# kubeflow/Code-Intelligence

Measured on AMD Instinct MI355X. Metric: LM tokens/sec (whole node), higher is better.
Workload: dtype bf16; 1 GPU; model=AWD-LSTM 4x2400 emb800 vocab60000, global_batch=512, seq_len=512, parallelism=dp1, device=MI355X

## Files before the change

code_intelligence_amd/ops/crossentropy.py:

```python
from __future__ import annotations

import os

import torch
from torch import Tensor

from . import extension as ext

__all__ = ["tied_decoder_ce", "TiedDecoderCE"]

_EMPTY = {}


def _empty_f32(device) -> Tensor:
    key = str(device)
    if key not in _EMPTY:
        _EMPTY[key] = torch.empty(0, dtype=torch.float32, device=device)
    return _EMPTY[key]


def _fp8r_enabled() -> bool:
    return os.environ.get("CI_CE_FP8R", "1") == "1"


_STORE = 448.0

_ce_side = None


def _ce_side_stream():
    global _ce_side
    if _ce_side is None:
        _ce_side = torch.cuda.Stream()
    return _ce_side


def _ce_overlap_enabled() -> bool:
    return os.environ.get("CI_CE_2STREAM", "0") == "1"


class _FusedCEFp8Function(torch.autograd.Function):

    @staticmethod
    def forward(ctx, h: Tensor, weight: Tensor, bias: Tensor, targets: Tensor):
        lib = ext.require()
        f8 = torch.float8_e4m3fn
        N, H = h.shape
        V = weight.shape[0]
        C = int(os.environ.get("CI_CE_CHUNK", _FusedCEFunction.CHUNK))
        dev = h.device
        lse = torch.empty(N, dtype=torch.float32, device=dev)
        tgt_logit = torch.empty(N, dtype=torch.float32, device=dev)
        b32 = bias.to(torch.float32) if bias is not None else _empty_f32(dev)
        tgt64 = targets.to(torch.int64)
        sa = (h.detach().abs().amax().float() / 448.0).clamp_min(1e-12)
        sw = (weight.detach().abs().amax().float() / 448.0).clamp_min(1e-12)
        h8 = torch.empty(h.shape, dtype=f8, device=dev)
        lib.quantize_e4m3(h.detach().contiguous(), h8, sa)
        w8 = torch.empty(weight.shape, dtype=f8, device=dev)
        lib.quantize_e4m3(weight.detach().contiguous(), w8, sw)
        w8_t = w8.t()
        w_t = weight.t()
        logits_full = None
        if os.environ.get("CI_CE_SAVE_LOGITS", "1") != "0":
            try:
                logits_full = torch.empty(N, V, dtype=h.dtype, device=dev)
            except torch.cuda.OutOfMemoryError:
                pass
        scratch = None if logits_full is not None else \
            torch.empty(min(C, N), V, dtype=h.dtype, device=dev)
        for s in range(0, N, C):
            e = min(N, s + C)
            logits = logits_full[s:e] if logits_full is not None \
                else scratch[: e - s]
            if (e - s) % 16 == 0 and H % 16 == 0 and V % 16 == 0:
                torch._scaled_mm(h8[s:e], w8_t, scale_a=sa, scale_b=sw,
                                 out_dtype=h.dtype, out=logits)
            else:
                torch.mm(h[s:e], w_t, out=logits)
            lib.ce_rowstats(logits, tgt64[s:e], b32, lse[s:e],
                            tgt_logit[s:e])
        wrows = weight.detach()[tgt64]
        tgt_logit = (h.detach() * wrows).sum(dim=1, dtype=torch.float32)
        if bias is not None:
            tgt_logit = tgt_logit + b32[tgt64]
        loss = (lse - tgt_logit).mean()
        ctx.save_for_backward(h, weight, b32, tgt64, lse, w8, sw)
        ctx.logits_full = logits_full
        ctx.has_bias = bias is not None
        ctx.bias_dtype = bias.dtype if bias is not None else None
        return loss

    @staticmethod
    def backward(ctx, dloss: Tensor):
        lib = ext.require()
        f8 = torch.float8_e4m3fn
        h, weight, b32, targets, lse, w8, sw = ctx.saved_tensors
        logits_full = ctx.logits_full
        ctx.logits_full = None
        has_bias = ctx.has_bias
        N, H = h.shape
        V = weight.shape[0]
        C = _FusedCEFunction.CHUNK
        dev = h.device
        dh = torch.empty_like(h)
        scale = (dloss / N).to(torch.float32).reshape(1)
        sc_over_store = (scale.reshape(()) / _STORE)
        scratch8 = torch.empty(min(C, N), V, dtype=f8, device=dev)
        Haug = H + 16 if has_bias else H
        h_aug = h
        if has_bias:
            h_aug = torch.zeros(N, Haug, dtype=h.dtype, device=dev)
            h_aug[:, :H] = h
            h_aug[:, H] = 1
        dw_aug = torch.zeros(V, Haug, dtype=torch.float32, device=dev)
        recompute = None if logits_full is not None else \
            torch.empty(min(C, N), V, dtype=h.dtype, device=dev)
        w8_cm = w8.t().contiguous().t()
        w_t = weight.t()
        bias_arg = b32 if has_bias else _empty_f32(dev)
        overlap = _ce_overlap_enabled() and logits_full is not None
        side = _ce_side_stream() if overlap else None
        main = torch.cuda.current_stream() if overlap else None
        for s in range(0, N, C):
            e = min(N, s + C)
            c = e - s
            if logits_full is not None:
                dlog = logits_full[s:e]
            else:
                dlog = recompute[:c]
                torch.mm(h[s:e], w_t, out=dlog)
            lib.ce_dlogits_dual(dlog, targets[s:e], bias_arg, lse[s:e],
                                scale, scratch8, _STORE)
            if c % 16 == 0 and H % 16 == 0 and V % 16 == 0:
                torch._scaled_mm(scratch8[:c], w8_cm, scale_a=sc_over_store,
                                 scale_b=sw, out_dtype=h.dtype, out=dh[s:e])
            else:
                torch.mm(dlog, weight, out=dh[s:e])
            if overlap:
                side.wait_stream(main)
                with torch.cuda.stream(side):
                    dw_aug += torch.mm(dlog.t(), h_aug[s:e])
            else:
                dw_aug += torch.mm(dlog.t(), h_aug[s:e])
        if overlap:
            main.wait_stream(side)
        dw = dw_aug[:, :H]
        db = dw_aug[:, H] if has_bias else None
        return (dh, dw.to(weight.dtype),
                db.to(ctx.bias_dtype) if has_bias else None, None)


class _FusedCEFunction(torch.autograd.Function):
    CHUNK = int(os.environ.get("CI_CE_CHUNK", "65536"))

    @staticmethod
    def forward(ctx, h: Tensor, weight: Tensor, bias: Tensor, targets: Tensor):
        lib = ext.require()
        N, H = h.shape
        V = weight.shape[0]
        C = int(os.environ.get("CI_CE_CHUNK", _FusedCEFunction.CHUNK))
        lse = torch.empty(N, dtype=torch.float32, device=h.device)
        tgt_logit = torch.empty(N, dtype=torch.float32, device=h.device)
        b32 = bias.to(torch.float32) if bias is not None else _empty_f32(h.device)
        tgt64 = targets.to(torch.int64)
        save_logits = os.environ.get("CI_CE_SAVE_LOGITS", "1") != "0"
        logits_full = None
        if save_logits:
            try:
                logits_full = torch.empty(N, V, dtype=h.dtype, device=h.device)
            except torch.cuda.OutOfMemoryError:
                logits_full = None
        scratch = None if logits_full is not None else \
            torch.empty(min(C, N), V, dtype=h.dtype, device=h.device)
        w_t = weight.t()
        for s in range(0, N, C):
            e = min(N, s + C)
            logits = logits_full[s:e] if logits_full is not None \
                else scratch[: e - s]
            torch.mm(h[s:e], w_t, out=logits)
            lib.ce_rowstats(logits, tgt64[s:e], b32, lse[s:e], tgt_logit[s:e])
        loss = (lse - tgt_logit).mean()
        ctx.save_for_backward(h, weight, b32, tgt64, lse)
        ctx.logits_full = logits_full
        ctx.has_bias = bias is not None
        ctx.bias_dtype = bias.dtype if bias is not None else None
        return loss

    @staticmethod
    def backward(ctx, dloss: Tensor):
        lib = ext.require()
        h, weight, b32, targets, lse = ctx.saved_tensors
        logits_full = ctx.logits_full
        ctx.logits_full = None
        has_bias = ctx.has_bias
        N, H = h.shape
        V = weight.shape[0]
        C = _FusedCEFunction.CHUNK
        dh = torch.empty_like(h)
        scale = (dloss / N).to(torch.float32).reshape(1)
        scratch = None if logits_full is not None else \
            torch.empty(min(C, N), V, dtype=h.dtype, device=h.device)
        w_t = weight.t()
        bias_arg = b32 if has_bias else _empty_f32(h.device)
        Haug = H + 16 if has_bias else H
        h_aug = h
        if has_bias:
            h_aug = torch.zeros(N, Haug, dtype=h.dtype, device=h.device)
            h_aug[:, :H] = h
            h_aug[:, H] = 1
        dw_aug = torch.zeros(V, Haug, dtype=torch.float32, device=h.device)
        for s in range(0, N, C):
            e = min(N, s + C)
            if logits_full is not None:
                dlog = logits_full[s:e]
            else:
                dlog = scratch[: e - s]
                torch.mm(h[s:e], w_t, out=dlog)
            lib.ce_dlogits(dlog, targets[s:e], bias_arg, lse[s:e], scale)
            torch.mm(dlog, weight, out=dh[s:e])
            dw_aug += torch.mm(dlog.t(), h_aug[s:e])
        dw = dw_aug[:, :H]
        db = dw_aug[:, H] if has_bias else None
        return (dh, dw.to(weight.dtype),
                db.to(ctx.bias_dtype) if has_bias else None, None)


@torch.no_grad()
def tied_decoder_accuracy(h: Tensor, weight: Tensor, bias: Tensor | None,
                          targets: Tensor, chunk: int = 16384) -> Tensor:
    h2 = h.reshape(-1, h.shape[-1])
    t2 = targets.reshape(-1)
    w_t = weight.t()
    correct = torch.zeros((), dtype=torch.long, device=h.device)
    for s in range(0, h2.shape[0], chunk):
        e = min(h2.shape[0], s + chunk)
        logits = torch.mm(h2[s:e], w_t)
        if bias is not None:
            logits += bias
        correct += (logits.argmax(dim=1) == t2[s:e]).sum()
    return correct.float() / max(1, h2.shape[0])


def tied_decoder_ce(h: Tensor, weight: Tensor, bias: Tensor | None,
                    targets: Tensor) -> Tensor:
    if h.is_cuda:
        if _fp8r_enabled() and h.dtype == torch.bfloat16 \
                and torch.is_grad_enabled() and h.requires_grad:
            return _FusedCEFp8Function.apply(h, weight, bias, targets)
        return _FusedCEFunction.apply(h, weight, bias, targets)
    logits = torch.nn.functional.linear(h.float(), weight.float(),
                                        bias.float() if bias is not None else None)
    return torch.nn.functional.cross_entropy(logits, targets)


class TiedDecoderCE(torch.nn.Module):

    def __init__(self, decoder: torch.nn.Linear):
        super().__init__()
        self.decoder = decoder

    def forward(self, h: Tensor, targets: Tensor) -> Tensor:
        return tied_decoder_ce(h.reshape(-1, h.shape[-1]), self.decoder.weight,
                               self.decoder.bias, targets.reshape(-1))
```

code_intelligence_amd/ops/csrc/bindings.cpp:

```cpp
#include <torch/extension.h>
#include <string>
#include <vector>

namespace ci {
void lstm_seq_forward_lib(at::Tensor xp, at::Tensor bias, at::Tensor h0,
                          at::Tensor c0, at::Tensor w_hh, at::Tensor hs,
                          at::Tensor cs, at::Tensor gates);
void lstm_seq_forward_fused(at::Tensor xp, at::Tensor bias, at::Tensor h0,
                            at::Tensor c0, at::Tensor w_hh, at::Tensor hs,
                            at::Tensor cs, at::Tensor gates);
void lstm_seq_forward_lib_fp8(at::Tensor xp, at::Tensor bias, at::Tensor h0,
                              at::Tensor c0, at::Tensor w8, at::Tensor wscale,
                              at::Tensor hs, at::Tensor cs, at::Tensor gates);
void quantize_e4m3(at::Tensor src, at::Tensor dst, at::Tensor scale);
void lstm_seq_forward_gemv(at::Tensor xp, at::Tensor bias, at::Tensor h0,
                           at::Tensor c0, at::Tensor w_hh, at::Tensor hs,
                           at::Tensor cs, at::Tensor gates);
long lstm_seq_forward_gemv_persistent(at::Tensor xp, at::Tensor bias,
                                      at::Tensor h0, at::Tensor c0,
                                      at::Tensor w_hh, at::Tensor hs,
                                      at::Tensor cs, at::Tensor gates,
                                      at::Tensor ws);
void lstm_seq_forward_gemv_fp8(at::Tensor xp, at::Tensor bias, at::Tensor h0,
                               at::Tensor c0, at::Tensor w8, at::Tensor wscale,
                               at::Tensor hs, at::Tensor cs, at::Tensor gates);
void lstm_seq_backward(at::Tensor dhs, at::Tensor dhT, at::Tensor dcT,
                       at::Tensor gates, at::Tensor hs, at::Tensor cs,
                       at::Tensor c0, at::Tensor w_hh, at::Tensor dgates,
                       at::Tensor dh0, at::Tensor dc0);
at::Tensor concat_pool(at::Tensor hidden, at::Tensor lengths);
std::vector<at::Tensor> qrnn_fo_pool_fwd(at::Tensor gates, at::Tensor c0);
std::vector<at::Tensor> qrnn_fo_pool_bwd(at::Tensor gates, at::Tensor c,
                                         at::Tensor c0, at::Tensor dh,
                                         at::Tensor dcT);
void ce_rowstats(at::Tensor logits, at::Tensor targets, at::Tensor bias,
                 at::Tensor lse, at::Tensor tgt);
void ce_dlogits(at::Tensor logits, at::Tensor targets, at::Tensor bias,
                at::Tensor lse, at::Tensor scale);
void ce_dlogits_dual(at::Tensor logits, at::Tensor targets, at::Tensor bias,
                     at::Tensor lse, at::Tensor scale, at::Tensor scratch8,
                     double store_scale);
at::Tensor artar_forward(at::Tensor out, at::Tensor r);
std::vector<at::Tensor> artar_backward(at::Tensor out, at::Tensor r,
                                       at::Tensor dloss, double ca, double cb);
void fused_adamw(std::vector<at::Tensor> params, std::vector<at::Tensor> grads,
                 std::vector<at::Tensor> masters, std::vector<at::Tensor> eas_,
                 std::vector<at::Tensor> eass, double lr, double b1, double b2,
                 double eps, double wd, double bc1, double bc2);
at::Tensor emb_gather(at::Tensor weight, at::Tensor ids, at::Tensor rowmask);
std::vector<std::string> tokenize_core(const std::string& text);
std::vector<std::vector<std::string>> tokenize_core_batch(
    const std::vector<std::string>& texts);
at::Tensor emb_scatter(at::Tensor gout, at::Tensor ids, at::Tensor rowmask,
                       long V, long pad_idx);
at::Tensor dropconnect_apply(at::Tensor w, long seed, double p);
void dropconnect_grad_(at::Tensor g, long seed, double p);
}

PYBIND11_MODULE(TORCH_EXTENSION_NAME, m) {
  m.def("lstm_seq_forward_lib", &ci::lstm_seq_forward_lib,
        "LSTM sequence forward (hipBLASLt GEMM + pointwise cell kernel)");
  m.def("lstm_seq_forward_fused", &ci::lstm_seq_forward_fused,
        "LSTM sequence forward (fused MFMA cell kernel)");
  m.def("lstm_seq_forward_lib_fp8", &ci::lstm_seq_forward_lib_fp8,
        "LSTM sequence forward (fp8 recurrent scaled_mm + pointwise cell)");
  m.def("quantize_e4m3", &ci::quantize_e4m3,
        "one-pass e4m3 quantize: dst = e4m3(src/scale)");
  m.def("lstm_seq_forward_gemv", &ci::lstm_seq_forward_gemv,
        "LSTM sequence forward (fused GEMV+cell kernel, small batch)");
  m.def("lstm_seq_forward_gemv_persistent",
        &ci::lstm_seq_forward_gemv_persistent,
        "whole-sequence persistent GEMV+cell kernel (grid barrier)");
  m.def("lstm_seq_forward_gemv_fp8", &ci::lstm_seq_forward_gemv_fp8,
        "LSTM sequence forward (fp8-weight GEMV+cell kernel)");
  m.def("lstm_seq_backward", &ci::lstm_seq_backward,
        "LSTM sequence backward (pointwise + per-step GEMM)");
  m.def("concat_pool", &ci::concat_pool, "masked mean/max/last concat pool");
  m.def("qrnn_fo_pool_fwd", &ci::qrnn_fo_pool_fwd,
        "QRNN fo-pool forward scan (activates gates in place)");
  m.def("qrnn_fo_pool_bwd", &ci::qrnn_fo_pool_bwd,
        "QRNN fo-pool backward scan (pre-activation gate grads)");
  m.def("ce_rowstats", &ci::ce_rowstats, "CE row logsumexp + target logit");
  m.def("ce_dlogits", &ci::ce_dlogits, "in-place (softmax-onehot)*scale");
  m.def("ce_dlogits_dual", &ci::ce_dlogits_dual,
        "in-place bf16 dlogits + e4m3 scratch copy for the fp8 dh GEMM");
  m.def("artar_forward", &ci::artar_forward,
        "fused AR/TAR partial sums (one pass over out and r)");
  m.def("artar_backward", &ci::artar_backward,
        "fused AR/TAR gradient kernel (dout and dr in one pass)");
  m.def("fused_adamw", &ci::fused_adamw, "fused AdamW step");
  m.def("emb_gather", &ci::emb_gather, "embedding gather with row dropout");
  m.def("tokenize_core", &ci::tokenize_core, "native ASCII tokenizer core");
  m.def("tokenize_core_batch", &ci::tokenize_core_batch,
        "native ASCII tokenizer core (batch, GIL released)");
  m.def("emb_scatter", &ci::emb_scatter, "embedding grad scatter-add");
  m.def("dropconnect_apply", &ci::dropconnect_apply,
        "seeded DropConnect mask-scale (no mask tensor)");
  m.def("dropconnect_grad_", &ci::dropconnect_grad_,
        "in-place seeded DropConnect grad mask");
}
```

code_intelligence_amd/ops/csrc/ce.hip:

```cpp
#include "common.h"

#include <hip/hip_fp8.h>

namespace ci {

typedef float f32x4 __attribute__((ext_vector_type(4)));

template <typename T, int VEC>
static __device__ __forceinline__ void load_vec(const T* p, float* out) {
  T buf[VEC];
  *reinterpret_cast<int4*>(buf) = *reinterpret_cast<const int4*>(p);
  #pragma unroll
  for (int e = 0; e < VEC; ++e) out[e] = ld(buf + e);
}

template <int VEC>
static __device__ __forceinline__ void load_bias(const float* b, float* out) {
  #pragma unroll
  for (int e = 0; e < VEC; e += 4)
    *reinterpret_cast<f32x4*>(out + e) = *reinterpret_cast<const f32x4*>(b + e);
}

template <typename T, int THREADS, bool HAS_BIAS>
__global__ void ce_rowstats_kernel(const T* __restrict__ logits, long row_stride,
                                   const long* __restrict__ targets,
                                   const float* __restrict__ bias,
                                   float* __restrict__ lse,
                                   float* __restrict__ tgt, int V) {
  constexpr int NW = THREADS / kWave;
  constexpr int VEC = 16 / sizeof(T);
  const int row = blockIdx.x;
  const T* x = logits + (long)row * row_stride;
  __shared__ float red_m[NW];
  __shared__ float red_s[NW];
  const int Vv = V / VEC * VEC;
  float v8[VEC], b8[VEC];
  float m = -3.4e38f, sum = 0.f;
  for (int v = threadIdx.x * VEC; v < Vv; v += THREADS * VEC) {
    load_vec<T, VEC>(x + v, v8);
    if (HAS_BIAS) {
      load_bias<VEC>(bias + v, b8);
      #pragma unroll
      for (int e = 0; e < VEC; ++e) v8[e] += b8[e];
    }
    float bm = v8[0];
    #pragma unroll
    for (int e = 1; e < VEC; ++e) bm = fmaxf(bm, v8[e]);
    if (bm > m) {
      sum *= __expf(m - bm);
      m = bm;
    }
    #pragma unroll
    for (int e = 0; e < VEC; ++e) sum += __expf(v8[e] - m);
  }
  for (int v = Vv + threadIdx.x; v < V; v += THREADS) {
    const float val = ld(x + v) + (HAS_BIAS ? bias[v] : 0.f);
    if (val > m) {
      sum *= __expf(m - val);
      m = val;
    }
    sum += __expf(val - m);
  }
  #pragma unroll
  for (int off = kWave / 2; off > 0; off >>= 1) {
    const float om = __shfl_down(m, off);
    const float os = __shfl_down(sum, off);
    const float nm = fmaxf(m, om);
    sum = sum * __expf(m - nm) + os * __expf(om - nm);
    m = nm;
  }
  if ((threadIdx.x & (kWave - 1)) == 0) {
    red_m[threadIdx.x / kWave] = m;
    red_s[threadIdx.x / kWave] = sum;
  }
  __syncthreads();
  if (threadIdx.x == 0) {
    float gm = red_m[0];
    for (int w = 1; w < NW; ++w) gm = fmaxf(gm, red_m[w]);
    float gs = 0.f;
    for (int w = 0; w < NW; ++w) gs += red_s[w] * __expf(red_m[w] - gm);
    lse[row] = gm + __logf(gs);
    tgt[row] = ld(x + targets[row]) + (HAS_BIAS ? bias[targets[row]] : 0.f);
  }
}

void ce_rowstats(at::Tensor logits, at::Tensor targets, at::Tensor bias,
                 at::Tensor lse, at::Tensor tgt) {
  CI_CHECK_CUDA(logits); CI_CHECK_CONTIG(logits);
  const int N = logits.size(0), V = logits.size(1);
  constexpr int THREADS = 256;
  const bool hb = bias.numel() > 0;
  CI_DISPATCH_FB(logits.scalar_type(), "ce_rowstats", [&] {
    if (hb) {
      hipLaunchKernelGGL((ce_rowstats_kernel<scalar_t, THREADS, true>), dim3(N),
          dim3(THREADS), 0, stream(),
          reinterpret_cast<const scalar_t*>(logits.data_ptr()), (long)V,
          targets.data_ptr<long>(), bias.data_ptr<float>(),
          lse.data_ptr<float>(), tgt.data_ptr<float>(), V);
    } else {
      hipLaunchKernelGGL((ce_rowstats_kernel<scalar_t, THREADS, false>), dim3(N),
          dim3(THREADS), 0, stream(),
          reinterpret_cast<const scalar_t*>(logits.data_ptr()), (long)V,
          targets.data_ptr<long>(), nullptr,
          lse.data_ptr<float>(), tgt.data_ptr<float>(), V);
    }
  });
}

template <typename T, int THREADS, bool HAS_BIAS>
__global__ void ce_dlogits_kernel(T* __restrict__ logits, long row_stride,
                                  const long* __restrict__ targets,
                                  const float* __restrict__ bias,
                                  const float* __restrict__ lse,
                                  const float* __restrict__ scale, int V) {
  constexpr int VEC = 16 / sizeof(T);
  const int row = blockIdx.x;
  T* x = logits + (long)row * row_stride;
  const float l = lse[row];
  const float sc = scale[0];
  const int tgt = (int)targets[row];
  const int Vv = V / VEC * VEC;
  float v8[VEC], b8[VEC];
  for (int v = threadIdx.x * VEC; v < Vv; v += THREADS * VEC) {
    load_vec<T, VEC>(x + v, v8);
    if (HAS_BIAS) {
      load_bias<VEC>(bias + v, b8);
      #pragma unroll
      for (int e = 0; e < VEC; ++e) v8[e] += b8[e];
    }
    T buf[VEC];
    #pragma unroll
    for (int e = 0; e < VEC; ++e) {
      float p = __expf(v8[e] - l);
      if (v + e == tgt) p -= 1.f;
      st(buf + e, p * sc);
    }
    *reinterpret_cast<int4*>(x + v) = *reinterpret_cast<const int4*>(buf);
  }
  for (int v = Vv + threadIdx.x; v < V; v += THREADS) {
    float p = __expf(ld(x + v) + (HAS_BIAS ? bias[v] : 0.f) - l);
    if (v == tgt) p -= 1.f;
    st(x + v, p * sc);
  }
}

void ce_dlogits(at::Tensor logits, at::Tensor targets, at::Tensor bias,
                at::Tensor lse, at::Tensor scale) {
  CI_CHECK_CUDA(logits); CI_CHECK_CONTIG(logits);
  const int N = logits.size(0), V = logits.size(1);
  constexpr int THREADS = 256;
  const bool hb = bias.numel() > 0;
  CI_DISPATCH_FB(logits.scalar_type(), "ce_dlogits", [&] {
    if (hb) {
      hipLaunchKernelGGL((ce_dlogits_kernel<scalar_t, THREADS, true>),
          dim3(N), dim3(THREADS), 0, stream(),
          reinterpret_cast<scalar_t*>(logits.data_ptr()), (long)V,
          targets.data_ptr<long>(), bias.data_ptr<float>(),
          lse.data_ptr<float>(), scale.data_ptr<float>(), V);
    } else {
      hipLaunchKernelGGL((ce_dlogits_kernel<scalar_t, THREADS, false>),
          dim3(N), dim3(THREADS), 0, stream(),
          reinterpret_cast<scalar_t*>(logits.data_ptr()), (long)V,
          targets.data_ptr<long>(), nullptr,
          lse.data_ptr<float>(), scale.data_ptr<float>(), V);
    }
  });
}

template <typename T, int THREADS, bool HAS_BIAS>
__global__ void ce_dlogits_dual_kernel(T* __restrict__ logits, long row_stride,
                                       const long* __restrict__ targets,
                                       const float* __restrict__ bias,
                                       const float* __restrict__ lse,
                                       const float* __restrict__ scale,
                                       unsigned char* __restrict__ scratch8,
                                       long srs, float store_scale, int V) {
  constexpr int VEC = 16 / sizeof(T);
  const int row = blockIdx.x;
  T* x = logits + (long)row * row_stride;
  unsigned char* s8 = scratch8 + (long)row * srs;
  const float l = lse[row];
  const float sc = scale[0];
  const int tgt = (int)targets[row];
  const int Vv = V / VEC * VEC;
  float v8[VEC], b8[VEC];
  for (int v = threadIdx.x * VEC; v < Vv; v += THREADS * VEC) {
    load_vec<T, VEC>(x + v, v8);
    if (HAS_BIAS) {
      load_bias<VEC>(bias + v, b8);
      #pragma unroll
      for (int e = 0; e < VEC; ++e) v8[e] += b8[e];
    }
    T buf[VEC];
    unsigned char q8[VEC];
    #pragma unroll
    for (int e = 0; e < VEC; ++e) {
      float p = __expf(v8[e] - l);
      if (v + e == tgt) p -= 1.f;
      st(buf + e, p * sc);
      q8[e] = __hip_fp8_e4m3(p * store_scale).__x;
    }
    *reinterpret_cast<int4*>(x + v) = *reinterpret_cast<const int4*>(buf);
    if constexpr (VEC == 8) {
      *reinterpret_cast<uint2*>(s8 + v) = *reinterpret_cast<const uint2*>(q8);
    } else {
      *reinterpret_cast<unsigned int*>(s8 + v) =
          *reinterpret_cast<const unsigned int*>(q8);
    }
  }
  for (int v = Vv + threadIdx.x; v < V; v += THREADS) {
    float p = __expf(ld(x + v) + (HAS_BIAS ? bias[v] : 0.f) - l);
    if (v == tgt) p -= 1.f;
    st(x + v, p * sc);
    s8[v] = __hip_fp8_e4m3(p * store_scale).__x;
  }
}

void ce_dlogits_dual(at::Tensor logits, at::Tensor targets, at::Tensor bias,
                     at::Tensor lse, at::Tensor scale, at::Tensor scratch8,
                     double store_scale) {
  CI_CHECK_CUDA(logits); CI_CHECK_CONTIG(logits); CI_CHECK_CONTIG(scratch8);
  const int N = logits.size(0), V = logits.size(1);
  TORCH_CHECK(scratch8.size(0) >= N && scratch8.size(1) == V,
              "ce_dlogits_dual: scratch too small");
  TORCH_CHECK(scratch8.scalar_type() == at::ScalarType::Byte ||
              scratch8.scalar_type() == at::ScalarType::Float8_e4m3fn);
  constexpr int THREADS = 256;
  const bool hb = bias.numel() > 0;
  CI_DISPATCH_FB(logits.scalar_type(), "ce_dlogits_dual", [&] {
    if (hb) {
      hipLaunchKernelGGL((ce_dlogits_dual_kernel<scalar_t, THREADS, true>),
          dim3(N), dim3(THREADS), 0, stream(),
          reinterpret_cast<scalar_t*>(logits.data_ptr()), (long)V,
          targets.data_ptr<long>(), bias.data_ptr<float>(),
          lse.data_ptr<float>(), scale.data_ptr<float>(),
          reinterpret_cast<unsigned char*>(scratch8.data_ptr()),
          (long)V, (float)store_scale, V);
    } else {
      hipLaunchKernelGGL((ce_dlogits_dual_kernel<scalar_t, THREADS, false>),
          dim3(N), dim3(THREADS), 0, stream(),
          reinterpret_cast<scalar_t*>(logits.data_ptr()), (long)V,
          targets.data_ptr<long>(), nullptr,
          lse.data_ptr<float>(), scale.data_ptr<float>(),
          reinterpret_cast<unsigned char*>(scratch8.data_ptr()),
          (long)V, (float)store_scale, V);
    }
  });
}

}
```

Before: 620,200 tokens/s.

## Fuse CE row logsumexp and dlogits into one forward pass with register-cached rows

Adds a kernel that reads each logits row once into registers, computes the logsumexp, and writes the bf16 dlogits in place along with an e4m3 copy during forward. The scale is 1/N, and the dloss multiply is deferred to the weight/bias gradients. Backward then skips the dlogits kernel and uses the stored fp8 buffer directly, removing a second full read/write pass over the N×V logits. In exchange it allocates an extra N×V fp8 buffer, uses heavy register caching (32 uint4 per thread) that may cut occupancy, and assumes dloss only scales the output. The dh GEMM still applies the dloss scale, while dw now gets it from an explicit post-multiply.

Measured after the change: 627,600 tokens/s, median of 6. 1.01x the previous value.

```diff
diff --git a/code_intelligence_amd/ops/crossentropy.py b/code_intelligence_amd/ops/crossentropy.py
--- a/code_intelligence_amd/ops/crossentropy.py
+++ b/code_intelligence_amd/ops/crossentropy.py
@@ -24,6 +24,8 @@
 
 
 _STORE = 448.0
+
+_ONEPASS_MAX_V = 256 * 32 * 8
 
 _ce_side = None
 
@@ -67,6 +69,18 @@
                 logits_full = torch.empty(N, V, dtype=h.dtype, device=dev)
             except torch.cuda.OutOfMemoryError:
                 pass
+        dlog8_full = None
+        if logits_full is not None and V <= _ONEPASS_MAX_V \
+                and H % 16 == 0 and V % 16 == 0 \
+                and N % 16 == 0 and min(C, N) % 16 == 0:
+            try:
+                dlog8_full = torch.empty(N, V, dtype=f8, device=dev)
+            except torch.cuda.OutOfMemoryError:
+                pass
+        onepass = dlog8_full is not None
+        if onepass:
+            inv_n = (torch.ones((), dtype=torch.float32, device=dev)
+                     / N).reshape(1)
         scratch = None if logits_full is not None else \
             torch.empty(min(C, N), V, dtype=h.dtype, device=dev)
         for s in range(0, N, C):
@@ -78,8 +92,12 @@
                                  out_dtype=h.dtype, out=logits)
             else:
                 torch.mm(h[s:e], w_t, out=logits)
-            lib.ce_rowstats(logits, tgt64[s:e], b32, lse[s:e],
-                            tgt_logit[s:e])
+            if onepass:
+                lib.ce_onepass_dual(logits, tgt64[s:e], b32, lse[s:e],
+                                    inv_n, dlog8_full[s:e], _STORE)
+            else:
+                lib.ce_rowstats(logits, tgt64[s:e], b32, lse[s:e],
+                                tgt_logit[s:e])
         wrows = weight.detach()[tgt64]
         tgt_logit = (h.detach() * wrows).sum(dim=1, dtype=torch.float32)
         if bias is not None:
@@ -87,6 +105,8 @@
         loss = (lse - tgt_logit).mean()
         ctx.save_for_backward(h, weight, b32, tgt64, lse, w8, sw)
         ctx.logits_full = logits_full
+        ctx.dlog8_full = dlog8_full
+        ctx.chunk = C
         ctx.has_bias = bias is not None
         ctx.bias_dtype = bias.dtype if bias is not None else None
         return loss
@@ -98,15 +118,19 @@
         h, weight, b32, targets, lse, w8, sw = ctx.saved_tensors
         logits_full = ctx.logits_full
         ctx.logits_full = None
+        dlog8_full = ctx.dlog8_full
+        ctx.dlog8_full = None
+        onepass = dlog8_full is not None
         has_bias = ctx.has_bias
         N, H = h.shape
         V = weight.shape[0]
-        C = _FusedCEFunction.CHUNK
+        C = ctx.chunk if onepass else _FusedCEFunction.CHUNK
         dev = h.device
         dh = torch.empty_like(h)
         scale = (dloss / N).to(torch.float32).reshape(1)
         sc_over_store = (scale.reshape(()) / _STORE)
-        scratch8 = torch.empty(min(C, N), V, dtype=f8, device=dev)
+        scratch8 = None if onepass else \
+            torch.empty(min(C, N), V, dtype=f8, device=dev)
         Haug = H + 16 if has_bias else H
         h_aug = h
         if has_bias:
@@ -130,10 +154,14 @@
             else:
                 dlog = recompute[:c]
                 torch.mm(h[s:e], w_t, out=dlog)
-            lib.ce_dlogits_dual(dlog, targets[s:e], bias_arg, lse[s:e],
-                                scale, scratch8, _STORE)
+            if onepass:
+                dlog8 = dlog8_full[s:e]
+            else:
+                lib.ce_dlogits_dual(dlog, targets[s:e], bias_arg, lse[s:e],
+                                    scale, scratch8, _STORE)
+                dlog8 = scratch8[:c]
             if c % 16 == 0 and H % 16 == 0 and V % 16 == 0:
-                torch._scaled_mm(scratch8[:c], w8_cm, scale_a=sc_over_store,
+                torch._scaled_mm(dlog8, w8_cm, scale_a=sc_over_store,
                                  scale_b=sw, out_dtype=h.dtype, out=dh[s:e])
             else:
                 torch.mm(dlog, weight, out=dh[s:e])
@@ -147,6 +175,12 @@
             main.wait_stream(side)
         dw = dw_aug[:, :H]
         db = dw_aug[:, H] if has_bias else None
+        if onepass:
+            dl = dloss.to(torch.float32)
+            dw_out = torch.empty(V, H, dtype=weight.dtype, device=dev)
+            torch.mul(dw, dl, out=dw_out)
+            return (dh, dw_out,
+                    (db * dl).to(ctx.bias_dtype) if has_bias else None, None)
         return (dh, dw.to(weight.dtype),
                 db.to(ctx.bias_dtype) if has_bias else None, None)
 
diff --git a/code_intelligence_amd/ops/csrc/bindings.cpp b/code_intelligence_amd/ops/csrc/bindings.cpp
--- a/code_intelligence_amd/ops/csrc/bindings.cpp
+++ b/code_intelligence_amd/ops/csrc/bindings.cpp
@@ -39,6 +39,9 @@
                 at::Tensor lse, at::Tensor scale);
 void ce_dlogits_dual(at::Tensor logits, at::Tensor targets, at::Tensor bias,
                      at::Tensor lse, at::Tensor scale, at::Tensor scratch8,
+                     double store_scale);
+void ce_onepass_dual(at::Tensor logits, at::Tensor targets, at::Tensor bias,
+                     at::Tensor lse, at::Tensor scale, at::Tensor out8,
                      double store_scale);
 at::Tensor artar_forward(at::Tensor out, at::Tensor r);
 std::vector<at::Tensor> artar_backward(at::Tensor out, at::Tensor r,
@@ -84,6 +87,8 @@
   m.def("ce_dlogits", &ci::ce_dlogits, "in-place (softmax-onehot)*scale");
   m.def("ce_dlogits_dual", &ci::ce_dlogits_dual,
         "in-place bf16 dlogits + e4m3 scratch copy for the fp8 dh GEMM");
+  m.def("ce_onepass_dual", &ci::ce_onepass_dual,
+        "one read of the row: lse + in-place bf16 dlogits + e4m3 copy");
   m.def("artar_forward", &ci::artar_forward,
         "fused AR/TAR partial sums (one pass over out and r)");
   m.def("artar_backward", &ci::artar_backward,
diff --git a/code_intelligence_amd/ops/csrc/ce.hip b/code_intelligence_amd/ops/csrc/ce.hip
--- a/code_intelligence_amd/ops/csrc/ce.hip
+++ b/code_intelligence_amd/ops/csrc/ce.hip
@@ -248,4 +248,185 @@
   });
 }
 
-}
+constexpr int kOnepassMaxVec = 32;
+
+static __device__ __forceinline__ void unpack_bf16x8(const uint4& c,
+                                                     float* out) {
+  out[0] = __uint_as_float(c.x << 16); out[1] = __uint_as_float(c.x & 0xffff0000u);
+  out[2] = __uint_as_float(c.y << 16); out[3] = __uint_as_float(c.y & 0xffff0000u);
+  out[4] = __uint_as_float(c.z << 16); out[5] = __uint_as_float(c.z & 0xffff0000u);
+  out[6] = __uint_as_float(c.w << 16); out[7] = __uint_as_float(c.w & 0xffff0000u);
+}
+
+template <int THREADS, bool HAS_BIAS>
+__global__ __launch_bounds__(THREADS) void ce_onepass_dual_kernel(
+    __hip_bfloat16* __restrict__ logits, long row_stride,
+    const long* __restrict__ targets, const float* __restrict__ bias,
+    float* __restrict__ lse, const float* __restrict__ scale,
+    unsigned char* __restrict__ out8, long srs, float store_scale, int V) {
+  #pragma clang fp contract(off)
+  using T = __hip_bfloat16;
+  constexpr int NW = THREADS / kWave;
+  constexpr int VEC = 8;
+  const int row = blockIdx.x;
+  T* x = logits + (long)row * row_stride;
+  unsigned char* s8 = out8 + (long)row * srs;
+  __shared__ float red_m[NW];
+  __shared__ float red_s[NW];
+  __shared__ float lse_sh;
+  const int Vv = V / VEC * VEC;
+  uint4 cache[kOnepassMaxVec];
+  #pragma unroll
+  for (int k = 0; k < kOnepassMaxVec; ++k) {
+    const int v = (threadIdx.x + k * THREADS) * VEC;
+    cache[k] = *reinterpret_cast<const uint4*>(x + min(v, Vv - VEC));
+  }
+  #pragma unroll
+  for (int k = 0; k < kOnepassMaxVec; ++k)
+    asm volatile("" : "+v"(cache[k].x), "+v"(cache[k].y), "+v"(cache[k].z),
+                      "+v"(cache[k].w));
+  float v8[VEC], b8[VEC];
+  float m = -3.4e38f, sum = 0.f;
+  #pragma unroll
+  for (int k = 0; k < kOnepassMaxVec; ++k) {
+    const int v = (threadIdx.x + k * THREADS) * VEC;
+    if (v < Vv) {
+      unpack_bf16x8(cache[k], v8);
+      if (HAS_BIAS) {
+        load_bias<VEC>(bias + v, b8);
+        #pragma unroll
+        for (int e = 0; e < VEC; ++e) v8[e] += b8[e];
+      }
+      float bm = v8[0];
+      #pragma unroll
+      for (int e = 1; e < VEC; ++e) bm = fmaxf(bm, v8[e]);
+      if (bm > m) {
+        sum *= __expf(m - bm);
+        m = bm;
+      }
+      #pragma unroll
+      for (int e = 0; e < VEC; ++e) sum += __expf(v8[e] - m);
+    }
+  }
+  for (int v = Vv + threadIdx.x; v < V; v += THREADS) {
+    const float val = ld(x + v) + (HAS_BIAS ? bias[v] : 0.f);
+    if (val > m) {
+      sum *= __expf(m - val);
+      m = val;
+    }
+    sum += __expf(val - m);
+  }
+  #pragma unroll
+  for (int off = kWave / 2; off > 0; off >>= 1) {
+    const float om = __shfl_down(m, off);
+    const float os = __shfl_down(sum, off);
+    const float nm = fmaxf(m, om);
+    const float t = os * __expf(om - nm);
+    sum = off > 1 ? __builtin_fmaf(sum, __expf(m - nm), t)
+                  : sum * __expf(m - nm) + t;
+    m = nm;
+  }
+  if ((threadIdx.x & (kWave - 1)) == 0) {
+    red_m[threadIdx.x / kWave] = m;
+    red_s[threadIdx.x / kWave] = sum;
+  }
+  __syncthreads();
+  if (threadIdx.x == 0) {
+    float gm = red_m[0];
+    for (int w = 1; w < NW; ++w) gm = fmaxf(gm, red_m[w]);
+    float gs = 0.f;
+    for (int w = 0; w < NW; ++w) gs += red_s[w] * __expf(red_m[w] - gm);
+    const float r = gm + __logf(gs);
+    lse[row] = r;
+    lse_sh = r;
+  }
+  __syncthreads();
+  #pragma unroll
+  for (int k = 0; k < kOnepassMaxVec; ++k)
+    asm volatile("" : "+v"(cache[k].x), "+v"(cache[k].y), "+v"(cache[k].z),
+                      "+v"(cache[k].w));
+  const float* bias2 = bias;
+  asm volatile("" : "+s"(bias2));
+  const float l = lse_sh;
+  const float sc = scale[0];
+  const int tgt = (int)targets[row];
+  #pragma unroll
+  for (int k = 0; k < kOnepassMaxVec; ++k) {
+    const int v = (threadIdx.x + k * THREADS) * VEC;
+    if (v < Vv) {
+      unpack_bf16x8(cache[k], v8);
+      if (HAS_BIAS) {
+        load_bias<VEC>(bias2 + v, b8);
+        #pragma unroll
+        for (int e = 0; e < VEC; ++e) v8[e] += b8[e];
+      }
+      T buf[VEC];
+      unsigned char q8[VEC];
+      #pragma unroll
+      for (int e = 0; e < VEC; ++e) {
+        float p = __expf(v8[e] - l);
+        if (v + e == tgt) p -= 1.f;
+        st(buf + e, p * sc);
+        q8[e] = __hip_fp8_e4m3(p * store_scale).__x;
+      }
+      *reinterpret_cast<int4*>(x + v) = *reinterpret_cast<const int4*>(buf);
+      *reinterpret_cast<uint2*>(s8 + v) = *reinterpret_cast<const uint2*>(q8);
+    }
+  }
+  for (int v = Vv + threadIdx.x; v < V; v += THREADS) {
+    float p = __expf(ld(x + v) + (HAS_BIAS ? bias2[v] : 0.f) - l);
+    if (v == tgt) p -= 1.f;
+    st(x + v, p * sc);
+    s8[v] = __hip_fp8_e4m3(p * store_scale).__x;
+  }
+}
+
+void ce_onepass_dual(at::Tensor logits, at::Tensor targets, at::Tensor bias,
+                     at::Tensor lse, at::Tensor scale, at::Tensor out8,
+                     double store_scale) {
+  CI_CHECK_CUDA(logits); CI_CHECK_CONTIG(logits); CI_CHECK_CONTIG(out8);
+  CI_CHECK_CUDA(targets); CI_CHECK_CUDA(lse); CI_CHECK_CUDA(scale);
+  CI_CHECK_CUDA(out8);
+  TORCH_CHECK(logits.dim() == 2 && out8.dim() == 2);
+  TORCH_CHECK(logits.scalar_type() == at::ScalarType::BFloat16,
+              "ce_onepass_dual: bf16 logits only");
+  constexpr int THREADS = 256;
+  const int N = logits.size(0), V = logits.size(1);
+  TORCH_CHECK(V >= 8, "ce_onepass_dual: V must hold one 16-byte vector");
+  TORCH_CHECK(V / 8 <= kOnepassMaxVec * THREADS,
+              "ce_onepass_dual: V=", V, " exceeds the register-cached row (",
+              kOnepassMaxVec * THREADS * 8, ")");
+  TORCH_CHECK(out8.size(0) >= N && out8.size(1) == V,
+              "ce_onepass_dual: fp8 output too small");
+  TORCH_CHECK(out8.scalar_type() == at::ScalarType::Byte ||
+              out8.scalar_type() == at::ScalarType::Float8_e4m3fn);
+  TORCH_CHECK(targets.scalar_type() == at::ScalarType::Long &&
+              targets.numel() >= N && lse.numel() >= N &&
+              lse.scalar_type() == at::ScalarType::Float &&
+              scale.scalar_type() == at::ScalarType::Float &&
+              scale.numel() >= 1);
+  const bool hb = bias.numel() > 0;
+  TORCH_CHECK(!hb || (bias.is_cuda() && bias.numel() >= V &&
+                      bias.scalar_type() == at::ScalarType::Float));
+  if (N == 0) return;
+  using T = __hip_bfloat16;
+  if (hb) {
+    hipLaunchKernelGGL((ce_onepass_dual_kernel<THREADS, true>),
+        dim3(N), dim3(THREADS), 0, stream(),
+        reinterpret_cast<T*>(logits.data_ptr()), (long)V,
+        targets.data_ptr<long>(), bias.data_ptr<float>(),
+        lse.data_ptr<float>(), scale.data_ptr<float>(),
+        reinterpret_cast<unsigned char*>(out8.data_ptr()),
+        (long)V, (float)store_scale, V);
+  } else {
+    hipLaunchKernelGGL((ce_onepass_dual_kernel<THREADS, false>),
+        dim3(N), dim3(THREADS), 0, stream(),
+        reinterpret_cast<T*>(logits.data_ptr()), (long)V,
+        targets.data_ptr<long>(), nullptr,
+        lse.data_ptr<float>(), scale.data_ptr<float>(),
+        reinterpret_cast<unsigned char*>(out8.data_ptr()),
+        (long)V, (float)store_scale, V);
+  }
+}
+
+}
```
